# baryshnikova-lab/safepy

Measured on AMD Instinct MI355X. Metric: node-attribute enrichments/sec (nodes x attrs x perms), compute_pvalues permutation test, higher is better.
Workload: dtype u1 (bit-sliced integer counts; f64 outputs)

## Files before the change

safepy_amd/csrc/attr.hip:

```cpp
#include "common.h"

template <typename T>
__device__ __forceinline__ double load_attr(const void *raw, int64_t idx) {
    return static_cast<double>(reinterpret_cast<const T *>(raw)[idx]);
}

template <typename T, int GC>
__global__ __launch_bounds__(256) void k_attr_stats(const void *__restrict__ raw, int64_t n, int64_t m,
                                                    int64_t rs, int64_t cs, unsigned int *__restrict__ row_bits,
                                                    unsigned long long *__restrict__ acc ,
                                                    double *__restrict__ col_sum, unsigned long long *__restrict__ max_abs_bits,
                                                    unsigned int *__restrict__ col_nan, int64_t rows_per_block) {
    extern __shared__ unsigned int s_bits[];
    constexpr int RL = 256 / GC;
    const int cx = GC == 1 ? 0 : (threadIdx.x & (GC - 1));
    const int ry = GC == 1 ? threadIdx.x : (threadIdx.x / GC);
    const int lane = threadIdx.x & 63;
    const int64_t j = static_cast<int64_t>(blockIdx.x) * GC + cx;
    const int64_t n_words = (n + 31) / 32;
    __shared__ double s_sum[256];
    __shared__ double s_max[256];
    __shared__ unsigned int s_nan[256], s_other[256], s_nonint[256];
    const int64_t r_begin = static_cast<int64_t>(blockIdx.y) * rows_per_block;
    const int64_t r_end = r_begin + rows_per_block < n ? r_begin + rows_per_block : n;
// ... 134 lines not shown
        const unsigned int o = __shfl_down(mx, off);
        mx = o > mx ? o : mx;
    }
    if ((threadIdx.x & 63) == 0) s_mx[threadIdx.x >> 6] = mx;
    if (threadIdx.x < 64) {
        unsigned long long a = acc[4 + threadIdx.x], b = acc[68 + threadIdx.x];
        for (int off = 32; off; off >>= 1) {
            a += __shfl_down(a, off);
            b += __shfl_down(b, off);
        }
        if (threadIdx.x == 0) s_fold[0] = a, s_fold[1] = b;
    }
    for (int64_t i = threadIdx.x; i < n; i += 256) bytes[i] = (bits[i >> 5] >> (i & 31)) & 1u;
    __syncthreads();
    if (threadIdx.x == 0) {
        const unsigned int m01 = s_mx[0] > s_mx[1] ? s_mx[0] : s_mx[1], m23 = s_mx[2] > s_mx[3] ? s_mx[2] : s_mx[3];
        tail[0] = acc[0] = s_fold[0];
        tail[1] = acc[1] = m01 > m23 ? m01 : m23;
        tail[2] = acc[2] = s_fold[1];
        tail[3] = acc[3];
    }
}

template <typename T>
__global__ __launch_bounds__(256) void k_fill_support(const void *__restrict__ raw, int64_t n, int64_t m, int64_t rs,
                                                      int64_t cs, const int32_t *__restrict__ sup_ptr,
                                                      int32_t *__restrict__ sup_row) {
    const int64_t j = (static_cast<int64_t>(blockIdx.x) * 256 + threadIdx.x) >> 6;
    const int lane = threadIdx.x & 63;
    if (j >= m) return;
    int32_t pos = sup_ptr[j];
    for (int64_t i0 = 0; i0 < n; i0 += 64) {
        const int64_t i = i0 + lane;
        const bool one = i < n && reinterpret_cast<const T *>(raw)[i * rs + j * cs] == static_cast<T>(1);
        const unsigned long long bal = __ballot(one);
        if (one) sup_row[pos + __popcll(bal & ((1ull << lane) - 1ull))] = static_cast<int32_t>(i);
        pos += __popcll(bal);
    }
}


template <typename T>
__global__ __launch_bounds__(256) void k_reindex_rows(const T *__restrict__ table, int64_t n_labels, int64_t m,
                                                      int64_t irs, int64_t ics, const int64_t *__restrict__ row_map,
                                                      T *__restrict__ out, int64_t n, int64_t ors, int64_t ocs, T fill) {
    __shared__ T tile[64][65];
// ... 73 lines not shown
    attr->h_sup_ptr.assign(m + 1, 0);
    int64_t total = 0;
    for (int64_t j = 0; j < m; ++j) {
        total += static_cast<int64_t>(sums[j]);
        SAFE_REQUIRE(total < (1ll << 31), "attr_build_support: too many ones for int32 offsets");
        attr->h_sup_ptr[j + 1] = static_cast<int32_t>(total);
    }
    attr->n_ones = total;
    SAFE_TRY(dev_alloc(&attr->sup_ptr, m + 1));
    SAFE_TRY(dev_alloc(&attr->sup_row, total));
    SAFE_HIP_CHECK(hipMemcpyAsync(attr->sup_ptr, attr->h_sup_ptr.data(), (m + 1) * sizeof(int32_t), hipMemcpyHostToDevice,
                                  ctx->stream));
    if (attr->dtype == SAFE_DTYPE_F32)
        hipLaunchKernelGGL(k_fill_support<float>, dim3(ceil_div(m * 64, 256)), dim3(256), 0, ctx->stream, attr->raw, n, m,
                           attr->row_stride, attr->col_stride, attr->sup_ptr, attr->sup_row);
    else
        hipLaunchKernelGGL(k_fill_support<double>, dim3(ceil_div(m * 64, 256)), dim3(256), 0, ctx->stream, attr->raw, n, m,
                           attr->row_stride, attr->col_stride, attr->sup_ptr, attr->sup_row);
    SAFE_HIP_CHECK(hipGetLastError());
    return SAFE_OK;
}

static size_t flags_block_bytes(int64_t n) { return static_cast<size_t>(ceil_div(n, 8)) * 8 + 32; }

int safe_attr_prepare(safe_attr *attr) {
    if (attr->stats_ready) return SAFE_OK;
    safe_ctx *ctx = attr->ctx;
    SAFE_HIP_CHECK(hipSetDevice(ctx->device));
    const int64_t n = attr->n, m = attr->m;
    const size_t flag_bytes = flags_block_bytes(n), tail_off = flag_bytes - 32;
    const int64_t n_words = (n + 31) / 32;
    SAFE_REQUIRE(n_words * sizeof(unsigned int) <= 150 * 1024, "safe_attr_stats: too many rows for the LDS row bitmap");
    void *tmp = nullptr;
    const size_t tmp_bytes = 132 * sizeof(unsigned long long) + static_cast<size_t>(n_words + m) * sizeof(unsigned int);
    SAFE_TRY(ctx_scratch(ctx, SCRATCH_ATTR_STATS, tmp_bytes, &tmp));
    unsigned long long *d_acc = static_cast<unsigned long long *>(tmp);
    unsigned int *d_rowbits = reinterpret_cast<unsigned int *>(d_acc + 132);
    unsigned int *d_colnan = d_rowbits + n_words;
    SAFE_HIP_CHECK(hipMemsetAsync(tmp, 0, tmp_bytes, ctx->stream));
    uint8_t *flags = nullptr;
    SAFE_TRY(ctx_block_alloc(ctx, flag_bytes, reinterpret_cast<void **>(&flags)));
    if (!attr->col_sum) SAFE_TRY(ctx_block_alloc(ctx, static_cast<size_t>(m) * sizeof(double), reinterpret_cast<void **>(&attr->col_sum)));
    const bool f32 = attr->dtype == SAFE_DTYPE_F32;
    const bool c_order = attr->col_stride == 1 && m > 1;
    if (c_order) SAFE_HIP_CHECK(hipMemsetAsync(attr->col_sum, 0, m * sizeof(double), ctx->stream));
#define STATS(T, GC, RPB)                                                                                          \
    do {                                                                                                           \
        if (n_words * sizeof(unsigned int) > 32 * 1024)                                                            \
            SAFE_HIP_CHECK(hipFuncSetAttribute(reinterpret_cast<const void *>(k_attr_stats<T, GC>),                \
                                               hipFuncAttributeMaxDynamicSharedMemorySize,                         \
                                               static_cast<int>(n_words * sizeof(unsigned int))));                 \
        hipLaunchKernelGGL((k_attr_stats<T, GC>), dim3(ceil_div(m, GC), ceil_div(n, RPB)), dim3(256),              \
                           n_words * sizeof(unsigned int), ctx->stream, attr->raw, n, m, attr->row_stride,         \
                           attr->col_stride, d_rowbits, d_acc, attr->col_sum, d_acc + 3, d_colnan,                 \
                           static_cast<int64_t>(RPB));                                                             \
    } while (0)
    if (c_order) {
        const int64_t groups = ceil_div(m, 64);
        const int64_t want_chunks = std::max<int64_t>(1, 2048 / groups);
        const int64_t rpb = std::max<int64_t>(256, ceil_div(ceil_div(n, want_chunks), 64) * 64);
        if (f32) STATS(float, 64, rpb);
        else STATS(double, 64, rpb);
    } else {
        if (f32) STATS(float, 1, n);
        else STATS(double, 1, n);
    }
#undef STATS
    hipLaunchKernelGGL(k_stats_finish, dim3(1), dim3(256), 0, ctx->stream, d_acc, d_colnan, m, d_rowbits, n, flags,
                       reinterpret_cast<unsigned long long *>(flags + tail_off));
    SAFE_HIP_CHECK(hipGetLastError());
    void *pinned = nullptr;
    SAFE_TRY(ctx_pinned(ctx, flag_bytes, &pinned));
    SAFE_HIP_CHECK(hipMemcpyAsync(pinned, flags, flag_bytes, hipMemcpyDeviceToHost, ctx->stream));
    SAFE_HIP_CHECK(safe_stream_sync(ctx->stream));
    const uint8_t *h_flags = static_cast<const uint8_t *>(pinned);
    unsigned long long h_acc[4];
    memcpy(h_acc, h_flags + tail_off, sizeof(h_acc));
    attr->n_other = static_cast<int64_t>(h_acc[0]);
    attr->max_nan_col = static_cast<int64_t>(h_acc[1]);
    attr->n_non_integer = static_cast<int64_t>(h_acc[2]);
    double mx;
    memcpy(&mx, &h_acc[3], sizeof(double));
    attr->max_abs = mx;
    if (!attr->flags_ready) {
        if (attr->row_flags) ctx_block_free(ctx, attr->row_flags, flag_bytes);
        attr->row_flags = flags;
        attr->flags_ready = true;
        int64_t cnt = 0;
        for (int64_t i = 0; i < n; ++i) cnt += h_flags[i] != 0;
        attr->n_rows_with_value = cnt;
        attr->h_row_flags.assign(h_flags, h_flags + n);
    } else {
        ctx_block_free(ctx, flags, flag_bytes);
    }
    attr->stats_ready = true;
    return SAFE_OK;
}

enum : unsigned int {
    CSC_PTR_FIRST = 1u,
// ... 369 lines not shown
    SAFE_HIP_CHECK(hipMemcpyAsync(h_acc, d_acc, sizeof(h_acc), hipMemcpyDeviceToHost, ctx->stream));
    SAFE_HIP_CHECK(safe_stream_sync(ctx->stream));
    if (n_nan) *n_nan = static_cast<int64_t>(h_acc[0]);
    if (n_zero) *n_zero = static_cast<int64_t>(h_acc[1]);
    if (n_positive) *n_positive = static_cast<int64_t>(h_acc[2]);
    if (n_negative) *n_negative = static_cast<int64_t>(h_acc[3]);
    return SAFE_OK;
}

int safe_attr_nan_to_zero(safe_attr *attr) {
    SAFE_REQUIRE(attr != nullptr, "safe_attr_nan_to_zero: attr is NULL");
    safe_ctx *ctx = attr->ctx;
    SAFE_HIP_CHECK(hipSetDevice(ctx->device));
    const int64_t count = attr->n * attr->m;
    const unsigned blocks = static_cast<unsigned>(std::min<int64_t>(ceil_div(count, 256), 8192));
    void *raw = const_cast<void *>(attr->raw);
    if (attr->dtype == SAFE_DTYPE_F32)
        hipLaunchKernelGGL(k_nan_to_zero<float>, dim3(blocks), dim3(256), 0, ctx->stream, reinterpret_cast<float *>(raw), count);
    else
        hipLaunchKernelGGL(k_nan_to_zero<double>, dim3(blocks), dim3(256), 0, ctx->stream, reinterpret_cast<double *>(raw), count);
    SAFE_HIP_CHECK(hipGetLastError());
    SAFE_HIP_CHECK(safe_stream_sync(ctx->stream));
    attr->stats_ready = false;
    attr->flags_ready = false;
    attr_free_support(attr);
    return SAFE_OK;
}

int safe_attr_download(safe_attr *attr, void *out_host) {
    SAFE_REQUIRE(attr && out_host, "safe_attr_download: NULL argument");
    safe_ctx *ctx = attr->ctx;
    SAFE_HIP_CHECK(hipSetDevice(ctx->device));
    const size_t bytes = static_cast<size_t>(attr->n) * attr->m * (attr->dtype == SAFE_DTYPE_F32 ? 4 : 8);
    SAFE_HIP_CHECK(hipMemcpyAsync(out_host, attr->raw, bytes, hipMemcpyDeviceToHost, ctx->stream));
    SAFE_HIP_CHECK(safe_stream_sync(ctx->stream));
    return SAFE_OK;
}

int safe_attr_destroy(safe_attr *attr) {
    if (!attr) return SAFE_OK;
    (void)hipSetDevice(attr->ctx->device);
    (void)safe_stream_sync(attr->ctx->stream);
    if (attr->owns_raw && attr->raw_pool_bytes) ctx_block_free(attr->ctx, const_cast<void *>(attr->raw), attr->raw_pool_bytes);
    else if (attr->owns_raw) (void)dev_free(attr->raw);
    ctx_block_free(attr->ctx, attr->row_flags, flags_block_bytes(attr->n));
    ctx_block_free(attr->ctx, attr->col_sum, static_cast<size_t>(attr->m) * sizeof(double));
    attr_free_support(attr);
    delete attr;
    return SAFE_OK;
}

int safe_attr_stats(safe_attr *attr, int64_t *n_other, int64_t *max_nan_col, int64_t *n_rows_with_value,
                    int64_t *n_non_integer) {
    SAFE_REQUIRE(attr != nullptr, "safe_attr_stats: attr is NULL");
    SAFE_TRY(safe_attr_prepare(attr));
    if (n_other) *n_other = attr->n_other;
    if (max_nan_col) *max_nan_col = attr->max_nan_col;
    if (n_rows_with_value) *n_rows_with_value = attr->n_rows_with_value;
    if (n_non_integer) *n_non_integer = attr->n_non_integer;
    return SAFE_OK;
}

int safe_attr_row_flags(safe_attr *attr, uint8_t *out_host) {
    SAFE_REQUIRE(attr && out_host, "safe_attr_row_flags: NULL argument");
    SAFE_TRY(safe_attr_prepare(attr));
    if (static_cast<int64_t>(attr->h_row_flags.size()) == attr->n) {
        memcpy(out_host, attr->h_row_flags.data(), attr->n);
        return SAFE_OK;
    }
// ... 39 lines not shown
```

safepy_amd/csrc/common.h:

```cpp
#pragma once
#include <hip/hip_runtime.h>

#include <algorithm>
#include <cstdarg>
#include <cmath>
#include <cstdint>
#include <cstdio>
#include <cstdlib>
#include <cstring>
#include <condition_variable>
#include <memory>
#include <mutex>
#include <atomic>
#include <string>
#include <thread>
#include <vector>

#include "safe_hip.h"
#include "bits_plan.h"

#define SAFE_WAVE 64
#define SAFE_PAD_U16 0xFFFFu

void safe_set_error(const char *fmt, ...);
// ... 362 lines not shown
    unsigned int *enriched;
    const double *nes_table;
    double nes_threshold;
    int sign_mode;
    int mode;
    int64_t ld;
};

struct safe_attr {
    safe_ctx *ctx = nullptr;
    int64_t n = 0, m = 0;
    int dtype = SAFE_DTYPE_F64;
    int64_t row_stride = 0, col_stride = 0;
    const void *raw = nullptr;
    bool owns_raw = false;
    size_t raw_pool_bytes = 0;
    uint8_t *row_flags = nullptr;
    std::vector<uint8_t> h_row_flags;
    bool flags_ready = false;
    bool stats_ready = false;
    int64_t n_other = 0, max_nan_col = 0, n_rows_with_value = 0, n_non_integer = 0;
    double *col_sum = nullptr;
    double max_abs = 0.0;
    int32_t *sup_ptr = nullptr;
    int32_t *sup_row = nullptr;
    int64_t n_ones = 0;
    std::vector<int32_t> h_sup_ptr;
    size_t sup_ptr_pool_bytes = 0, sup_row_pool_bytes = 0;
};

struct DrawStream;

struct safe_perms {
    safe_ctx *ctx = nullptr;
    int64_t n = 0;
    int64_t count = 0;
    int64_t k = 0;
    std::vector<int32_t> h_movable;
    DrawStream *stream = nullptr;
    int64_t generated = 0, enqueued = 0;
    std::vector<int64_t> stages;
    std::vector<hipEvent_t> chunk_done;
    std::vector<uint32_t> h_local;
    std::thread drawer;
    bool on_worker = false;
    bool worker_done = false;
    bool twin = false;
    bool on_worker2 = false, worker_done2 = false;
    DrawStream *stream2 = nullptr;
    void *h_stage2[3] = {nullptr, nullptr, nullptr};
    hipEvent_t staged2[3] = {nullptr, nullptr, nullptr};
    std::vector<uint32_t> h_local2;
// ... 104 lines not shown
```

safepy_amd/csrc/enrich.hip:

```cpp
#include <algorithm>
#include <cmath>
#include <numeric>

#include "common.h"
#include "hyp_math.h"

template <typename T, int BN, int PLANES>
__global__ __launch_bounds__(256) void k_tile_prep(const void *__restrict__ raw, int64_t n, int64_t rs, int64_t cs,
                                                   int64_t col0, int64_t mloc, int64_t n_tiles,
                                                   double *__restrict__ bt) {
    const int64_t idx = static_cast<int64_t>(blockIdx.x) * 256 + threadIdx.x;
    const int64_t total = n_tiles * (n + 1) * BN;
    if (idx >= total) return;
    const int c = static_cast<int>(idx % BN);
    const int64_t row = (idx / BN) % (n + 1);
    const int64_t tile = idx / (static_cast<int64_t>(BN) * (n + 1));
    const int64_t j = tile * BN + c;
    double v = 0.0, v2 = 0.0, nn = 0.0;
    if (row < n && j < mloc) {
        const T x = reinterpret_cast<const T *>(raw)[row * rs + (col0 + j) * cs];
        if (x == x) {
            v = static_cast<double>(x);
            v2 = static_cast<double>(static_cast<T>(x * x));
            nn = 1.0;
// ... 1151 lines not shown
                                         uint32_t (&l1)[CL]) {
    blk_task_core<LV, CL, DBG>(obs, perm_ids, perm_stride, lane, nblk, np, g0, g1, l0, l1);
}

template <int LV>
__device__ __forceinline__ void observed_wave(const u32x4 *__restrict__ ids, int lane, int nblk, uint32_t *__restrict__ obs,
                                              uint32_t (&oo0)[BT_LV], uint32_t (&oo1)[BT_LV]) {
    uint32_t o0[LV], o1[LV];
    blk_sum<LV, 2, 1>(ids, lane, nblk, o0, o1);
#pragma unroll
    for (int l = 0; l < BT_LV; ++l) {
        oo0[l] = l < LV ? o0[l < LV ? l : 0] : 0u;
        oo1[l] = l < LV ? o1[l < LV ? l : 0] : 0u;
        obs[l * 64 + lane] = oo0[l];
        obs[(BT_LV + l) * 64 + lane] = oo1[l];
    }
}

__global__ __launch_bounds__(256) void k_bits_observed(int64_t n, const int32_t *__restrict__ sell_row,
                                                       const int64_t *__restrict__ slice_off,
                                                       const int32_t *__restrict__ slice_width,
                                                       const uint16_t *__restrict__ sell_col2b, int64_t n_slices,
                                                       const uint2 *__restrict__ bbits, int64_t mloc,
                                                       uint32_t *__restrict__ obs, double *__restrict__ ns_out) {
    extern __shared__ unsigned int lds[];
    uint2 *T = reinterpret_cast<uint2 *>(lds);
    if ((uint32_t)(uintptr_t)((__attribute__((address_space(3))) unsigned int *)lds) != 0u) __builtin_trap();
    const int wave = __builtin_amdgcn_readfirstlane(threadIdx.x >> 6), lane = threadIdx.x & 63;
    const int64_t wg = blockIdx.x, s = static_cast<int64_t>(blockIdx.y) * 4 + wave;
    load_word_column(T, bbits + wg * (n + 1), n);
    __syncthreads();
    if (s >= n_slices) return;
    const int wdt = __builtin_amdgcn_readfirstlane(slice_width[s]);
    const u32x4 *ids = reinterpret_cast<const u32x4 *>(sell_col2b) + slice_off[s] / 8;
    uint32_t *my_obs = obs + (wg * n_slices + s) * (2 * BT_LV * 64);
    uint32_t oo0[BT_LV], oo1[BT_LV];
    if (wdt <= 8) observed_wave<4>(ids, lane, wdt >> 3, my_obs, oo0, oo1);
    else if (wdt <= 56) observed_wave<6>(ids, lane, wdt >> 3, my_obs, oo0, oo1);
    else if (wdt <= 248) observed_wave<8>(ids, lane, wdt >> 3, my_obs, oo0, oo1);
    else if (wdt <= 504) observed_wave<9>(ids, lane, wdt >> 3, my_obs, oo0, oo1);
    else observed_wave<BT_LV>(ids, lane, wdt >> 3, my_obs, oo0, oo1);
    if (ns_out) {
        const int32_t row = sell_row[s * 64 + lane];
        uint16_t *tile = reinterpret_cast<uint16_t *>(lds + 2 * ((n + 2) & ~int64_t(1)) + 4) + wave * (64 * 66);
#pragma unroll
        for (int half = 0; half < 2; ++half)
#pragma unroll
            for (int bit = 0; bit < 32; ++bit)
                tile[lane * 66 + half * 32 + bit] = static_cast<uint16_t>(half ? vextract<BT_LV>(oo1, bit) : vextract<BT_LV>(oo0, bit));
        const int64_t jc = wg * 64 + lane;
#pragma unroll 8
        for (int r = 0; r < 64; ++r) {
// ... 327 lines not shown
    const int64_t j = wg * 64 + lane;
    bool one = false;
    if (r < n && j < mloc) one = reinterpret_cast<const T *>(raw)[r * rs + (col0 + j) * cs] == static_cast<T>(1);
    const unsigned long long w = __builtin_amdgcn_ballot_w64(one);
    if (lane == 0) bbits[wg * (n + 1) + r] = make_uint2(static_cast<uint32_t>(w), static_cast<uint32_t>(w >> 32));
}

static void launch_bits_prep(safe_ctx *ctx, const safe_attr *attr, int64_t col0, int64_t mloc, int64_t n_wg, uint2 *d_bits) {
    const int64_t n = attr->n;
    const bool f32 = attr->dtype == SAFE_DTYPE_F32;
    if (attr->col_stride == 1 && attr->row_stride != 1) {
        const dim3 grid(n_wg, ceil_div(n + 1, 4)), block(256);
        if (f32) hipLaunchKernelGGL(k_bits_prep_rowmajor<float>, grid, block, 0, ctx->stream, attr->raw, n, attr->row_stride,
                                    attr->col_stride, col0, mloc, n_wg, d_bits);
        else hipLaunchKernelGGL(k_bits_prep_rowmajor<double>, grid, block, 0, ctx->stream, attr->raw, n, attr->row_stride,
                                attr->col_stride, col0, mloc, n_wg, d_bits);
    } else {
        const dim3 grid(ceil_div(n_wg * (n + 1), 256)), block(256);
        if (f32) hipLaunchKernelGGL(k_bits_prep<float>, grid, block, 0, ctx->stream, attr->raw, n, attr->row_stride,
                                    attr->col_stride, col0, mloc, n_wg, d_bits);
        else hipLaunchKernelGGL(k_bits_prep<double>, grid, block, 0, ctx->stream, attr->raw, n, attr->row_stride,
                                attr->col_stride, col0, mloc, n_wg, d_bits);
    }
}


template <bool TABLE>
__global__ __launch_bounds__(64) void k_counts_bits(const int32_t *__restrict__ sell_row,
                                                    const int64_t *__restrict__ slice_off,
                                                    const int32_t *__restrict__ slice_width,
                                                    const int32_t *__restrict__ sell_col, int64_t n,
                                                    const uint2 *__restrict__ bbits, int64_t mloc,
                                                    double *__restrict__ out, HypLookup hl) {
    const int64_t s = blockIdx.x, wg = blockIdx.y;
    const int lane = threadIdx.x;
    const int32_t row = sell_row[s * 64 + lane];
    const int32_t *cols = sell_col + slice_off[s] + lane;
    const int wdt = slice_width[s];
    const uint2 *T = bbits + wg * (n + 1);
    uint32_t s0[BT_LV], s1[BT_LV];
#pragma unroll
    for (int l = 0; l < BT_LV; ++l) s0[l] = s1[l] = 0;
    for (int t0 = 0; t0 < wdt; t0 += 8) {
        uint32_t x0[8], x1[8];
#pragma unroll
        for (int u = 0; u < 8; ++u) {
// ... 593 lines not shown
constexpr int BITS_NS = 2;

struct BitsBuffers {
    uint2 *d_bits = nullptr;
    int4 *d_tasks = nullptr;
    unsigned int *d_queue = nullptr, *d_gl = nullptr;
    int64_t n_pad = 0, entries_pad = 0;
    uint16_t *d_ids[BITS_NS] = {nullptr, nullptr};
    uint16_t *d_ids_tail = nullptr;
    uint32_t *d_obs = nullptr;
};
static int bits_call_buffers(safe_ctx *ctx, const safe_nbr *nbr, const BitsForm &form, const BitsTail &tail, int64_t mloc, int64_t span,
                             int64_t tail_span, BitsBuffers *b) {
    const size_t n_task = bits_plan_records(nbr->bits_plan, form).size();
    const int64_t n_launch = tail.n_major + tail.n_chunks;
    void *ws = nullptr;
    SAFE_TRY(ctx_scratch(ctx, SCRATCH_TASKS, n_task * sizeof(int4) + (8 * n_launch + 4) * sizeof(unsigned int), &ws));
    b->d_tasks = static_cast<int4 *>(ws);
    b->d_queue = reinterpret_cast<unsigned int *>(b->d_tasks + n_task);
    b->n_pad = nbr->n_slices * 64;
    SAFE_TRY(ctx_scratch(ctx, SCRATCH_COUNTERS, static_cast<size_t>(b->n_pad) * mloc * sizeof(unsigned int), reinterpret_cast<void **>(&b->d_gl)));
    SAFE_HIP_CHECK(hipMemcpyAsync(b->d_tasks, nbr->bits_plan_pinned, n_task * sizeof(int4), hipMemcpyHostToDevice, ctx->stream));
    SAFE_HIP_CHECK(hipMemsetAsync(b->d_queue, 0, 8 * n_launch * sizeof(unsigned int), ctx->stream));
    SAFE_HIP_CHECK(hipMemsetAsync(b->d_gl, 0, static_cast<size_t>(b->n_pad) * mloc * sizeof(unsigned int), ctx->stream));
    safe_trace("launch_bits: buffers ready");
    b->entries_pad = (nbr->sell_entries + 1024 + 255) / 256 * 256;
    for (int s = 0; s < BITS_NS; ++s)
        SAFE_TRY(ctx_scratch(ctx, scratch_pair(SCRATCH_STREAM_A, s), static_cast<size_t>(span) * b->entries_pad * sizeof(uint16_t), reinterpret_cast<void **>(&b->d_ids[s])));
    if (tail.n_chunks)
        SAFE_TRY(ctx_scratch(ctx, SCRATCH_BITS_TAIL_IDS, static_cast<size_t>(tail_span) * b->entries_pad * sizeof(uint16_t), reinterpret_cast<void **>(&b->d_ids_tail)));
    return SAFE_OK;
}

static int bits_observe(safe_ctx *ctx, const safe_nbr *nbr, const BitsForm &form, int64_t mloc, double *ns_out, BitsBuffers *b) {
    const int64_t n_wg = ceil_div(mloc, 64);
    SAFE_TRY(ctx_scratch(ctx, SCRATCH_BITS_OBSERVED, static_cast<size_t>(n_wg) * nbr->n_slices * 2 * BT_LV * 64 * sizeof(uint32_t),
                         reinterpret_cast<void **>(&b->d_obs)));
    const size_t lds_obs = form.lds_bytes + (ns_out ? 4 * 64 * 66 * sizeof(uint16_t) : 0);
    SAFE_HIP_CHECK(hipFuncSetAttribute(reinterpret_cast<const void *>(k_bits_observed), hipFuncAttributeMaxDynamicSharedMemorySize,
                                       static_cast<int>(lds_obs)));
    hipLaunchKernelGGL(k_bits_observed, dim3(n_wg, ceil_div(nbr->n_slices, 4)), dim3(256), lds_obs, ctx->stream, nbr->n, nbr->sell_row,
                       nbr->slice_off, nbr->slice_width, nbr->sell_col2b, nbr->n_slices, b->d_bits, mloc, b->d_obs, ns_out);
    SAFE_HIP_CHECK(hipGetLastError());
    return SAFE_OK;
}

static int bits_tail_lists(safe_ctx *ctx, const safe_nbr *nbr, safe_perms *perms, const std::vector<int64_t> &starts, const BitsTail &tail,
                           const BitsBuffers &b, hipEvent_t *plain) {
    hipStream_t tail_ps = ctx->more_streams[1], kstreams[BITS_NS] = {ctx->stream, ctx->side_stream};
    const int64_t n_stage = static_cast<int64_t>(starts.size()) - 1, entries_pad = b.entries_pad;
    SAFE_HIP_CHECK(hipStreamWaitEvent(tail_ps, plain[0], 0));
    for (int64_t t = tail.n_major; t < n_stage; ++t) {
        SAFE_TRY(perms_wait(perms, starts[t + 1], tail_ps));
        hipLaunchKernelGGL(k_permute_cols, dim3(ceil_div(entries_pad, 4096), starts[t + 1] - starts[t]), dim3(256),
                           static_cast<size_t>(perms->stride16) * sizeof(uint16_t), tail_ps, perms->table16, perms->stride16,
                           nbr->sell_col2b, nbr->sell_entries, entries_pad, starts[t], starts[t + 1] - starts[t],
                           static_cast<uint32_t>(8 * nbr->n), b.d_ids_tail + (starts[t] - tail.p_split) * entries_pad, 3);
        SAFE_HIP_CHECK(hipGetLastError());
    }
    SAFE_HIP_CHECK(hipEventRecord(plain[8], tail_ps));
    for (int s = 0; s < BITS_NS; ++s) {
        SAFE_HIP_CHECK(hipEventRecord(plain[4 + s], kstreams[s]));
        SAFE_HIP_CHECK(hipStreamWaitEvent(kstreams[s], plain[8], 0));
    }
    return SAFE_OK;
// ... 37 lines not shown
        }
        const int64_t grid = std::min<int64_t>(n_tasks, grid_max);
        unsigned int *queue_c = b.d_queue + 8 * c;
        const uint16_t *ids_c = in_tail ? b.d_ids_tail : b.d_ids[c % BITS_NS];
        BitsQueues bq = blk ? plan.wave_queues[list] : plan.list_queues[list];
        void *blk_args[] = {(void *)&n, (void *)&ids_c, (void *)&entries_pad, (void *)&nbr->sell_row, (void *)&nbr->slice_off,
                            (void *)&nbr->slice_width, (void *)&b.d_obs, (void *)&nbr->n_slices, (void *)&b.d_bits, (void *)&bq,
                            (void *)&d_tasks, (void *)&p_base, (void *)&p_limit, (void *)&queue_c, (void *)&mloc, (void *)&b.d_gl,
                            (void *)&n_pad};
        void *pre_args[] = {(void *)&n, (void *)&ids_c, (void *)&entries_pad, (void *)&nbr->sell_row, (void *)&nbr->slice_off,
                            (void *)&nbr->slice_width, (void *)&nbr->sell_col2, (void *)&nbr->n_slices, (void *)&b.d_bits, (void *)&n_tasks,
                            (void *)&d_tasks, (void *)&p_base, (void *)&p_limit, (void *)&queue_c, (void *)&mloc, (void *)&b.d_gl,
                            (void *)&n_pad, (void *)&ns_out};
        SAFE_HIP_CHECK(hipLaunchKernel(kfn, dim3(grid), dim3(form.block), blk ? blk_args : pre_args, form.lds_bytes, ks));
        if (in_tail) chunk_final(c, ks);
        SAFE_HIP_CHECK(hipGetLastError());
        SAFE_HIP_CHECK(hipEventRecord(fr.ev[2 * c + 1], ks));
    }
    return SAFE_OK;
}

static int launch_bits(safe_ctx *ctx, safe_nbr *nbr, safe_attr *attr, safe_perms *perms, int64_t col0, int64_t col1,
                       const PermOut &out) {
    const int64_t n = nbr->n, mloc = col1 - col0, n_wg = ceil_div(mloc, 64), P = perms->count;
    const BitsForm form = bits_form(n, nbr->max_count, nbr->sell_col2 != nullptr, 160 * 1024);
    SAFE_REQUIRE(form.kind != BITS_NONE, "launch_bits: no bit-sliced form for %lld nodes with neighborhoods of up to %lld members",
                 static_cast<long long>(n), static_cast<long long>(nbr->max_count));
    safe_trace("launch_bits: enter");
    BitsBuffers b;
    SAFE_TRY(ctx_scratch(ctx, SCRATCH_OPERANDS, static_cast<size_t>(n_wg) * (n + 1) * sizeof(uint2), reinterpret_cast<void **>(&b.d_bits)));
    launch_bits_prep(ctx, attr, col0, mloc, n_wg, b.d_bits);
    safe_trace("launch_bits: prep launched");
    const BitsSwitches sw = bits_switches(ctx);
    int64_t span = 1;
    const std::vector<int64_t> starts = perm_launch_starts(perms, &span, 1, sw.tail_frac > 0.0);
    ctx->xc_made = 0;
    const BitsTail tail = bits_tail_split(ctx->xc_want, ctx->xc_cols, safe_ctx::XC_MAX, form.kind == BITS_BLK, starts, P, mloc, sw.tail_frac);
    const int64_t n_tail = tail.n_chunks, tail_span = P - tail.p_split;
    const int64_t n_launch = tail.n_major + n_tail;
    const int per_cu = static_cast<int>(std::max<size_t>(1, std::min<size_t>(8, (160 * 1024) / bits_lds_bytes(n, perms->stride16))));
    SAFE_TRY(bits_task_plan(ctx, nbr, form, tail, starts, static_cast<int64_t>(ctx->num_cu) * per_cu, mloc));
    safe_trace("launch_bits: tasks built");
    SAFE_TRY(bits_call_buffers(ctx, nbr, form, tail, mloc, span, tail_span, &b));
    const void *kfn = bits_form_kernel(form, sw.dbg);
    if (!kfn) return SAFE_E_INVALID;
    SAFE_HIP_CHECK(hipFuncSetAttribute(kfn, hipFuncAttributeMaxDynamicSharedMemorySize, static_cast<int>(form.lds_bytes)));
    if (form.kind == BITS_BLK) SAFE_TRY(bits_observe(ctx, nbr, form, mloc, out.ns, &b));
    for (int64_t k = 0; k < n_tail; ++k)
        if (!ctx->xc_events[k]) SAFE_HIP_CHECK(hipEventCreateWithFlags(&ctx->xc_events[k], hipEventDisableTiming));
    SpanFrame fr;
    SAFE_TRY(span_frame_open(ctx, form.kind == BITS_BLK ? "k_permtest_bits_blk" : "k_permtest_bits_pre", n_launch, 12, &fr));
    int xc_rc = SAFE_OK;
    SAFE_TRY(bits_launch_spans(ctx, nbr, perms, form, kfn, starts, tail, b, mloc, out.ns, fr, &xc_rc));
    ctx->packed_counts = b.d_gl;
// ... 3 lines not shown
    ctx->packed_layout = 0;
    SAFE_REQUIRE(xc_rc == SAFE_OK, "launch_bits: recording a column chunk's event failed");
    if (n_tail) {
        ctx->xc_made = static_cast<int>(n_tail);
        ctx->xc_tail_perms = tail_span;
        for (int64_t k = 0; k <= n_tail; ++k) ctx->xc_bounds[k] = std::min<int64_t>(k * ctx->xc_cols, mloc);
        ctx->xc_bounds[n_tail] = mloc;
        safe_trace("launch_bits: column chunks enqueued");
        if (ctx->xc_callback) ctx->xc_callback(ctx->xc_user);
    }
    SAFE_TRY(span_frame_join(ctx, fr));
    SAFE_TRY(enrich_finalize_counts(ctx, b.d_gl, b.n_pad, nbr->sell_row, mloc, P, out, nullptr));
    SAFE_HIP_CHECK(hipGetLastError());
    safe_trace("launch_bits: all enqueued");
    SAFE_TRY(span_frame_close(ctx, fr));
    safe_trace("launch_bits: synced");
    if (sw.dbg & 128) blk_trace_dump(static_cast<int>(n_launch));
    return SAFE_OK;
}

static int launch_counts_bits(safe_ctx *ctx, safe_nbr *nbr, safe_attr *attr, int64_t col0, int64_t col1, double *out_dev) {
    const int64_t n = nbr->n, mloc = col1 - col0, n_wg = ceil_div(mloc, 64);
    uint2 *d_bits = nullptr;
    SAFE_TRY(ctx_scratch(ctx, SCRATCH_OPERANDS, static_cast<size_t>(n_wg) * (n + 1) * sizeof(uint2), reinterpret_cast<void **>(&d_bits)));
    launch_bits_prep(ctx, attr, col0, mloc, n_wg, d_bits);
    SAFE_HIP_CHECK(hipEventRecord(ctx->k0, ctx->stream));
    hipLaunchKernelGGL(k_counts_bits<false>, dim3(nbr->n_slices, n_wg), dim3(64), 0, ctx->stream, nbr->sell_row, nbr->slice_off,
                       nbr->slice_width, nbr->sell_col, n, d_bits, mloc, out_dev, HypLookup{});
    SAFE_HIP_CHECK(hipGetLastError());
    SAFE_HIP_CHECK(hipEventRecord(ctx->k1, ctx->stream));
    ctx->last_kernel.name = "k_counts_bits";
    return SAFE_OK;
}

static size_t ldsf64_bytes(int64_t n, int64_t stride16) {
    return (8 * static_cast<size_t>(n + 1) + static_cast<size_t>(stride16) + 4) * sizeof(unsigned int);
}

static int launch_lds_f64(safe_ctx *ctx, safe_nbr *nbr, safe_attr *attr, safe_perms *perms, int64_t col0, int64_t col1,
                          bool z, const PermOut &out_in) {
    const int64_t n = nbr->n, mloc = col1 - col0, P = perms->count;
    const int64_t n_tiles = z ? mloc : ceil_div(mloc, 4);
    PermOut out = out_in;
    double *d_tiles = nullptr, *d_ns = out.ns;
    SAFE_TRY(ctx_scratch(ctx, SCRATCH_OPERANDS, static_cast<size_t>(n_tiles) * (n + 1) * 4 * sizeof(double), reinterpret_cast<void **>(&d_tiles)));
    if (!d_ns) SAFE_TRY(ctx_scratch(ctx, SCRATCH_F64_MATRIX, static_cast<size_t>(n) * mloc * sizeof(double), reinterpret_cast<void **>(&d_ns)));
    {
        const dim3 grid(ceil_div(n_tiles * (n + 1), 256)), block(256);
// ... 121 lines not shown
    hl.kid = d_kid;
    hl.tab = d_tab;
    hl.n_kid = n_kid;
    hl.xs = xs;
    hl.p_cut = p_cut;
    SAFE_TRY(ctx_scratch(ctx, SCRATCH_HYP_DUMMY, 64 * sizeof(double), reinterpret_cast<void **>(&hl.dummy)));
    hl.pvalues_pos = p_dev;
    hl.nes = nes_dev;
    hl.nes_binary = nb_dev;
    hl.enriched = d_enr;
    if (split) {
        int rc = mfma_counts_split_emit(ctx, nbr, split, hl);
        if (rc == SAFE_OK && enriched_f64) {
            hipLaunchKernelGGL(k_u32_to_f64, dim3(ceil_div(mloc, 256)), dim3(256), 0, ctx->stream, d_enr, enriched_f64, mloc);
            if (hipGetLastError() != hipSuccess) rc = SAFE_E_HIP;
        }
        (void)safe_stream_sync(hs);
        (void)hipEventDestroy(ids_done);
        SAFE_TRY(rc);
    } else if (use_mfma) {
        SAFE_TRY(launch_mfma_counts(ctx, nbr, attr, col0, col1, hl));
    } else {
        uint2 *d_bits = nullptr;
        SAFE_TRY(ctx_scratch(ctx, SCRATCH_OPERANDS, static_cast<size_t>(n_wg) * (n + 1) * sizeof(uint2), reinterpret_cast<void **>(&d_bits)));
        launch_bits_prep(ctx, attr, col0, mloc, n_wg, d_bits);
        SAFE_HIP_CHECK(hipEventRecord(ctx->k0, ctx->stream));
        hipLaunchKernelGGL(k_counts_bits<true>, dim3(nbr->n_slices, n_wg), dim3(64), 0, ctx->stream, nbr->sell_row, nbr->slice_off,
                           nbr->slice_width, nbr->sell_col, n, d_bits, mloc, static_cast<double *>(nullptr), hl);
        SAFE_HIP_CHECK(hipGetLastError());
        SAFE_HIP_CHECK(hipEventRecord(ctx->k1, ctx->stream));
        ctx->last_kernel.name = "k_counts_bits<hypergeom>";
    }
    if (split && enriched_f64 && enriched_done) *enriched_done = true;
    SAFE_HIP_CHECK(safe_stream_sync(ctx->stream));
    *fused = true;
    return SAFE_OK;
}

__global__ __launch_bounds__(256) void k_counts_to_outputs(const double *__restrict__ counts_neg, const double *__restrict__ counts_pos,
                                                           const double *__restrict__ ns, int64_t total, int64_t m, int64_t n_perm,
                                                           PermOut out) {
    const int64_t idx = static_cast<int64_t>(blockIdx.x) * 256 + threadIdx.x;
    if (idx >= total) return;
    const double qnan = __longlong_as_double(0x7FF8000000000000ll);
    bool obs_nan = ns && ns[idx] != ns[idx];
    const double cn = counts_neg[idx], cp = counts_pos[idx], Pd = static_cast<double>(n_perm);
    if (!obs_nan && !(cn >= 0.0 && cn <= Pd && cp >= 0.0 && cp <= Pd)) {
        atomicOr(&out.enriched[m], 1u);
// ... 545 lines not shown
```

Measured before the change: 6851 billion.

## Build attribute bit planes during stats pass and reuse them in counting kernels

Adds a kernel that, in one sweep over the raw attribute matrix, computes the column/row stats and also writes the packed 64-column bit planes used by the bit-sliced counting kernels. Those planes are cached on the attribute and reused by the counting paths, which skip their own prep pass over the raw data when the planes are valid and aligned. It also drops a separate memset of the global counter buffer by having the observed-count kernel zero it. The cost is extra device memory for the cached planes (capped at 8 MB). When non-binary values are found, the old stats kernel runs as a fallback, so the raw matrix is read twice in that case.

Measured after the change: 6900 billion, median of 6. Within noise of the previous version (+0.7%).

```diff
diff --git a/safepy_amd/csrc/attr.hip b/safepy_amd/csrc/attr.hip
--- a/safepy_amd/csrc/attr.hip
+++ b/safepy_amd/csrc/attr.hip
@@ -180,6 +180,125 @@
     }
 }
 
+template <typename T, bool ROWMAJOR>
+__global__ __launch_bounds__(256) void k_attr_planes(const T *__restrict__ raw, int64_t n, int64_t m, int64_t rs, int64_t cs,
+                                                     uint2 *__restrict__ bits, unsigned int *__restrict__ row_bits,
+                                                     unsigned long long *__restrict__ acc ,
+                                                     unsigned int *__restrict__ col_nan, unsigned int *__restrict__ col_ones) {
+    __shared__ unsigned int s_ones[64], s_nan[64];
+    const int lane = threadIdx.x & 63, wave = threadIdx.x >> 6;
+    const int64_t wg = blockIdx.x, j0 = wg * 64;
+    const int64_t r0 = static_cast<int64_t>(blockIdx.y) * 256 + wave * 64;
+    const int n_col = static_cast<int>(m - j0 < 64 ? m - j0 : 64);
+    if (threadIdx.x < 64) s_ones[threadIdx.x] = s_nan[threadIdx.x] = 0;
+    __syncthreads();
+    unsigned int my_ones = 0, my_nan = 0;
+    unsigned int n_other = 0;
+    unsigned long long has = 0;
+    uint32_t w[2] = {0, 0};
+    if (!ROWMAJOR) {
+        const int64_t r = r0 + lane;
+        const bool live = r < n;
+        bool any = false;
+        const T *src = raw + (live ? r : 0) * rs + j0 * cs;
+        auto tally = [&](int a, T x) {
+            const bool one = x == static_cast<T>(1), nan = x != x;
+            const unsigned int c1 = __popcll(__ballot(one)), cn = __popcll(__ballot(nan));
+            n_other += __popcll(__ballot(!(one || nan || x == static_cast<T>(0))));
+            if (one) (a < 32 ? w[0] : w[1]) |= 1u << (a & 31);
+            any |= live && !nan;
+            if (lane == a) my_ones += c1, my_nan += cn;
+        };
+        if (r0 < n && n_col == 64) {
+#pragma unroll
+            for (int a0 = 0; a0 < 64; a0 += 16) {
+                T x[16];
+#pragma unroll
+                for (int u = 0; u < 16; ++u) x[u] = live ? src[(a0 + u) * cs] : static_cast<T>(0);
+#pragma unroll
+                for (int u = 0; u < 16; ++u) tally(a0 + u, x[u]);
+            }
+        } else if (r0 < n) {
+            for (int a = 0; a < n_col; ++a) tally(a, live ? src[a * cs] : static_cast<T>(0));
+        }
+        has = __ballot(any);
+    } else {
+        const int64_t j = j0 + lane;
+        const bool col_live = lane < n_col;
+#pragma unroll 1
+        for (int k0 = 0; k0 < 64 && r0 + k0 < n; k0 += 16) {
+            T x[16];
+#pragma unroll
+            for (int u = 0; u < 16; ++u) {
+                const int64_t r = r0 + k0 + u;
+                x[u] = col_live && r < n ? raw[r * rs + j * cs] : static_cast<T>(0);
+            }
+#pragma unroll
+            for (int u = 0; u < 16; ++u) {
+                const int k = k0 + u;
+                const bool live = col_live && r0 + k < n;
+                const bool one = x[u] == static_cast<T>(1), nan = x[u] != x[u];
+                const unsigned long long b1 = __ballot(one);
+                n_other += __popcll(__ballot(!(one || nan || x[u] == static_cast<T>(0))));
+                if (__ballot(live && !nan)) has |= 1ull << k;
+                my_ones += one;
+                my_nan += nan;
+                if (lane == k) w[0] = static_cast<uint32_t>(b1), w[1] = static_cast<uint32_t>(b1 >> 32);
+            }
+        }
+    }
+    if (r0 + lane <= n) bits[wg * (n + 1) + r0 + lane] = make_uint2(w[0], w[1]);
+    if (lane == 0) {
+        const unsigned int lo = static_cast<unsigned int>(has), hi = static_cast<unsigned int>(has >> 32);
+        if (lo && (lo & ~row_bits[r0 >> 5])) atomicOr(&row_bits[r0 >> 5], lo);
+        if (hi && (hi & ~row_bits[(r0 >> 5) + 1])) atomicOr(&row_bits[(r0 >> 5) + 1], hi);
+        if (n_other) atomicAdd(&acc[4 + (wg & 63)], static_cast<unsigned long long>(n_other));
+    }
+    if (my_ones) atomicAdd(&s_ones[lane], my_ones);
+    if (my_nan) atomicAdd(&s_nan[lane], my_nan);
+    __syncthreads();
+    if (threadIdx.x < n_col) {
+        if (s_ones[threadIdx.x]) atomicAdd(&col_ones[j0 + threadIdx.x], s_ones[threadIdx.x]);
+        if (s_nan[threadIdx.x]) atomicAdd(&col_nan[j0 + threadIdx.x], s_nan[threadIdx.x]);
+    }
+}
+
+__global__ __launch_bounds__(256) void k_planes_finish(unsigned long long *__restrict__ acc, const unsigned int *__restrict__ col_nan,
+                                                       const unsigned int *__restrict__ col_ones, int64_t m, double *__restrict__ col_sum,
+                                                       const unsigned int *__restrict__ bits, int64_t n, uint8_t *__restrict__ bytes,
+                                                       unsigned long long *__restrict__ tail) {
+    __shared__ unsigned int s_mx[4], s_any[4];
+    __shared__ unsigned long long s_fold;
+    unsigned int mx = 0, any = 0;
+    for (int64_t i = threadIdx.x; i < m; i += 256) {
+        const unsigned int ones = col_ones[i];
+        mx = col_nan[i] > mx ? col_nan[i] : mx;
+        any |= ones;
+        col_sum[i] = static_cast<double>(ones);
+    }
+    for (int off = 32; off; off >>= 1) {
+        const unsigned int o = __shfl_down(mx, off);
+        mx = o > mx ? o : mx;
+        any |= __shfl_down(any, off);
+    }
+    if ((threadIdx.x & 63) == 0) s_mx[threadIdx.x >> 6] = mx, s_any[threadIdx.x >> 6] = any;
+    if (threadIdx.x < 64) {
+        unsigned long long a = acc[4 + threadIdx.x];
+        for (int off = 32; off; off >>= 1) a += __shfl_down(a, off);
+        if (threadIdx.x == 0) s_fold = a;
+    }
+    for (int64_t i = threadIdx.x; i < n; i += 256) bytes[i] = (bits[i >> 5] >> (i & 31)) & 1u;
+    __syncthreads();
+    if (threadIdx.x == 0) {
+        const unsigned int m01 = s_mx[0] > s_mx[1] ? s_mx[0] : s_mx[1], m23 = s_mx[2] > s_mx[3] ? s_mx[2] : s_mx[3];
+        const double mxabs = (s_any[0] | s_any[1] | s_any[2] | s_any[3]) ? 1.0 : 0.0;
+        tail[0] = acc[0] = s_fold;
+        tail[1] = acc[1] = m01 > m23 ? m01 : m23;
+        tail[2] = acc[2] = 0;
+        tail[3] = acc[3] = static_cast<unsigned long long>(__double_as_longlong(mxabs));
+    }
+}
+
 template <typename T>
 __global__ __launch_bounds__(256) void k_fill_support(const void *__restrict__ raw, int64_t n, int64_t m, int64_t rs,
                                                       int64_t cs, const int32_t *__restrict__ sup_ptr,
@@ -299,6 +418,10 @@
 }
 
 static size_t flags_block_bytes(int64_t n) { return static_cast<size_t>(ceil_div(n, 8)) * 8 + 32; }
+static size_t attr_plane_bytes(const safe_attr *attr) {
+    return static_cast<size_t>(ceil_div(attr->m, 64)) * static_cast<size_t>(attr->n + 1) * sizeof(uint2);
+}
+constexpr size_t ATTR_PLANES_POOL_MAX = size_t(8) << 20;
 
 int safe_attr_prepare(safe_attr *attr) {
     if (attr->stats_ready) return SAFE_OK;
@@ -309,50 +432,80 @@
     const int64_t n_words = (n + 31) / 32;
     SAFE_REQUIRE(n_words * sizeof(unsigned int) <= 150 * 1024, "safe_attr_stats: too many rows for the LDS row bitmap");
     void *tmp = nullptr;
-    const size_t tmp_bytes = 132 * sizeof(unsigned long long) + static_cast<size_t>(n_words + m) * sizeof(unsigned int);
+    const size_t tmp_bytes = 132 * sizeof(unsigned long long) + static_cast<size_t>(n_words + 2 * m) * sizeof(unsigned int);
     SAFE_TRY(ctx_scratch(ctx, SCRATCH_ATTR_STATS, tmp_bytes, &tmp));
     unsigned long long *d_acc = static_cast<unsigned long long *>(tmp);
     unsigned int *d_rowbits = reinterpret_cast<unsigned int *>(d_acc + 132);
     unsigned int *d_colnan = d_rowbits + n_words;
-    SAFE_HIP_CHECK(hipMemsetAsync(tmp, 0, tmp_bytes, ctx->stream));
+    unsigned int *d_colones = d_colnan + m;
     uint8_t *flags = nullptr;
     SAFE_TRY(ctx_block_alloc(ctx, flag_bytes, reinterpret_cast<void **>(&flags)));
     if (!attr->col_sum) SAFE_TRY(ctx_block_alloc(ctx, static_cast<size_t>(m) * sizeof(double), reinterpret_cast<void **>(&attr->col_sum)));
     const bool f32 = attr->dtype == SAFE_DTYPE_F32;
     const bool c_order = attr->col_stride == 1 && m > 1;
-    if (c_order) SAFE_HIP_CHECK(hipMemsetAsync(attr->col_sum, 0, m * sizeof(double), ctx->stream));
-#define STATS(T, GC, RPB)                                                                                          \
-    do {                                                                                                           \
-        if (n_words * sizeof(unsigned int) > 32 * 1024)                                                            \
-            SAFE_HIP_CHECK(hipFuncSetAttribute(reinterpret_cast<const void *>(k_attr_stats<T, GC>),                \
-                                               hipFuncAttributeMaxDynamicSharedMemorySize,                         \
-                                               static_cast<int>(n_words * sizeof(unsigned int))));                 \
-        hipLaunchKernelGGL((k_attr_stats<T, GC>), dim3(ceil_div(m, GC), ceil_div(n, RPB)), dim3(256),              \
-                           n_words * sizeof(unsigned int), ctx->stream, attr->raw, n, m, attr->row_stride,         \
-                           attr->col_stride, d_rowbits, d_acc, attr->col_sum, d_acc + 3, d_colnan,                 \
-                           static_cast<int64_t>(RPB));                                                             \
-    } while (0)
-    if (c_order) {
-        const int64_t groups = ceil_div(m, 64);
-        const int64_t want_chunks = std::max<int64_t>(1, 2048 / groups);
-        const int64_t rpb = std::max<int64_t>(256, ceil_div(ceil_div(n, want_chunks), 64) * 64);
-        if (f32) STATS(float, 64, rpb);
-        else STATS(double, 64, rpb);
-    } else {
-        if (f32) STATS(float, 1, n);
-        else STATS(double, 1, n);
-    }
-#undef STATS
-    hipLaunchKernelGGL(k_stats_finish, dim3(1), dim3(256), 0, ctx->stream, d_acc, d_colnan, m, d_rowbits, n, flags,
-                       reinterpret_cast<unsigned long long *>(flags + tail_off));
-    SAFE_HIP_CHECK(hipGetLastError());
     void *pinned = nullptr;
     SAFE_TRY(ctx_pinned(ctx, flag_bytes, &pinned));
-    SAFE_HIP_CHECK(hipMemcpyAsync(pinned, flags, flag_bytes, hipMemcpyDeviceToHost, ctx->stream));
-    SAFE_HIP_CHECK(safe_stream_sync(ctx->stream));
     const uint8_t *h_flags = static_cast<const uint8_t *>(pinned);
     unsigned long long h_acc[4];
-    memcpy(h_acc, h_flags + tail_off, sizeof(h_acc));
+    attr->bits_ready = false;
+    const size_t plane_bytes = attr_plane_bytes(attr);
+    bool swept = false;
+    if (plane_bytes <= ATTR_PLANES_POOL_MAX) {
+        if (!attr->bits) SAFE_TRY(ctx_block_alloc(ctx, plane_bytes, reinterpret_cast<void **>(&attr->bits)));
+        SAFE_HIP_CHECK(hipMemsetAsync(tmp, 0, tmp_bytes, ctx->stream));
+        const dim3 grid(static_cast<unsigned int>(ceil_div(m, 64)), static_cast<unsigned int>(ceil_div(n + 1, 256)));
+#define PLANES(T, RM)                                                                                                      \
+    hipLaunchKernelGGL((k_attr_planes<T, RM>), grid, dim3(256), 0, ctx->stream, static_cast<const T *>(attr->raw), n, m,   \
+                       attr->row_stride, attr->col_stride, attr->bits, d_rowbits, d_acc, d_colnan, d_colones)
+        if (attr->col_stride == 1 && attr->row_stride != 1) {
+            if (f32) PLANES(float, true);
+            else PLANES(double, true);
+        } else {
+            if (f32) PLANES(float, false);
+            else PLANES(double, false);
+        }
+#undef PLANES
+        hipLaunchKernelGGL(k_planes_finish, dim3(1), dim3(256), 0, ctx->stream, d_acc, d_colnan, d_colones, m, attr->col_sum, d_rowbits, n,
+                           flags, reinterpret_cast<unsigned long long *>(flags + tail_off));
+        SAFE_HIP_CHECK(hipGetLastError());
+        SAFE_HIP_CHECK(hipMemcpyAsync(pinned, flags, flag_bytes, hipMemcpyDeviceToHost, ctx->stream));
+        SAFE_HIP_CHECK(safe_stream_sync(ctx->stream));
+        memcpy(h_acc, h_flags + tail_off, sizeof(h_acc));
+        swept = h_acc[0] == 0;
+    }
+    if (!swept) {
+        SAFE_HIP_CHECK(hipMemsetAsync(tmp, 0, tmp_bytes, ctx->stream));
+        if (c_order) SAFE_HIP_CHECK(hipMemsetAsync(attr->col_sum, 0, m * sizeof(double), ctx->stream));
+#define STATS(T, GC, RPB)                                                                                          \
+        do {                                                                                                       \
+            if (n_words * sizeof(unsigned int) > 32 * 1024)                                                        \
+                SAFE_HIP_CHECK(hipFuncSetAttribute(reinterpret_cast<const void *>(k_attr_stats<T, GC>),            \
+                                                   hipFuncAttributeMaxDynamicSharedMemorySize,                     \
+                                                   static_cast<int>(n_words * sizeof(unsigned int))));             \
+            hipLaunchKernelGGL((k_attr_stats<T, GC>), dim3(ceil_div(m, GC), ceil_div(n, RPB)), dim3(256),          \
+                               n_words * sizeof(unsigned int), ctx->stream, attr->raw, n, m, attr->row_stride,     \
+                               attr->col_stride, d_rowbits, d_acc, attr->col_sum, d_acc + 3, d_colnan,             \
+                               static_cast<int64_t>(RPB));                                                         \
+        } while (0)
+        if (c_order) {
+            const int64_t groups = ceil_div(m, 64);
+            const int64_t want_chunks = std::max<int64_t>(1, 2048 / groups);
+            const int64_t rpb = std::max<int64_t>(256, ceil_div(ceil_div(n, want_chunks), 64) * 64);
+            if (f32) STATS(float, 64, rpb);
+            else STATS(double, 64, rpb);
+        } else {
+            if (f32) STATS(float, 1, n);
+            else STATS(double, 1, n);
+        }
+#undef STATS
+        hipLaunchKernelGGL(k_stats_finish, dim3(1), dim3(256), 0, ctx->stream, d_acc, d_colnan, m, d_rowbits, n, flags,
+                           reinterpret_cast<unsigned long long *>(flags + tail_off));
+        SAFE_HIP_CHECK(hipGetLastError());
+        SAFE_HIP_CHECK(hipMemcpyAsync(pinned, flags, flag_bytes, hipMemcpyDeviceToHost, ctx->stream));
+        SAFE_HIP_CHECK(safe_stream_sync(ctx->stream));
+        memcpy(h_acc, h_flags + tail_off, sizeof(h_acc));
+    }
+    attr->bits_ready = swept;
     attr->n_other = static_cast<int64_t>(h_acc[0]);
     attr->max_nan_col = static_cast<int64_t>(h_acc[1]);
     attr->n_non_integer = static_cast<int64_t>(h_acc[2]);
@@ -768,6 +921,7 @@
     SAFE_HIP_CHECK(hipGetLastError());
     SAFE_HIP_CHECK(safe_stream_sync(ctx->stream));
     attr->stats_ready = false;
+    attr->bits_ready = false;
     attr->flags_ready = false;
     attr_free_support(attr);
     return SAFE_OK;
@@ -791,6 +945,7 @@
     else if (attr->owns_raw) (void)dev_free(attr->raw);
     ctx_block_free(attr->ctx, attr->row_flags, flags_block_bytes(attr->n));
     ctx_block_free(attr->ctx, attr->col_sum, static_cast<size_t>(attr->m) * sizeof(double));
+    ctx_block_free(attr->ctx, attr->bits, attr_plane_bytes(attr));
     attr_free_support(attr);
     delete attr;
     return SAFE_OK;
diff --git a/safepy_amd/csrc/common.h b/safepy_amd/csrc/common.h
--- a/safepy_amd/csrc/common.h
+++ b/safepy_amd/csrc/common.h
@@ -408,12 +408,18 @@
     int64_t n_other = 0, max_nan_col = 0, n_rows_with_value = 0, n_non_integer = 0;
     double *col_sum = nullptr;
     double max_abs = 0.0;
+    uint2 *bits = nullptr;
+    bool bits_ready = false;
     int32_t *sup_ptr = nullptr;
     int32_t *sup_row = nullptr;
     int64_t n_ones = 0;
     std::vector<int32_t> h_sup_ptr;
     size_t sup_ptr_pool_bytes = 0, sup_row_pool_bytes = 0;
 };
+static inline uint2 *attr_bits_planes(const safe_attr *a, int64_t col0, int64_t col1) {
+    if (!a->bits_ready || !a->bits || col0 % 64 != 0 || !(col1 == a->m || col1 % 64 == 0)) return nullptr;
+    return a->bits + (col0 / 64) * (a->n + 1);
+}
 
 struct DrawStream;
 
diff --git a/safepy_amd/csrc/enrich.hip b/safepy_amd/csrc/enrich.hip
--- a/safepy_amd/csrc/enrich.hip
+++ b/safepy_amd/csrc/enrich.hip
@@ -1197,12 +1197,19 @@
                                                        const int32_t *__restrict__ slice_width,
                                                        const uint16_t *__restrict__ sell_col2b, int64_t n_slices,
                                                        const uint2 *__restrict__ bbits, int64_t mloc,
-                                                       uint32_t *__restrict__ obs, double *__restrict__ ns_out) {
+                                                       uint32_t *__restrict__ obs, double *__restrict__ ns_out,
+                                                       unsigned int *__restrict__ gl_clear) {
     extern __shared__ unsigned int lds[];
     uint2 *T = reinterpret_cast<uint2 *>(lds);
     if ((uint32_t)(uintptr_t)((__attribute__((address_space(3))) unsigned int *)lds) != 0u) __builtin_trap();
     const int wave = __builtin_amdgcn_readfirstlane(threadIdx.x >> 6), lane = threadIdx.x & 63;
     const int64_t wg = blockIdx.x, s = static_cast<int64_t>(blockIdx.y) * 4 + wave;
+    if (gl_clear && s < n_slices) {
+        const int64_t n_pad = n_slices * 64;
+        const int n_col = static_cast<int>(mloc - wg * 64 < 64 ? mloc - wg * 64 : 64);
+        unsigned int *p = gl_clear + wg * 64 * n_pad + s * 64 + lane;
+        for (int c = 0; c < n_col; ++c) p[c * n_pad] = 0u;
+    }
     load_word_column(T, bbits + wg * (n + 1), n);
     __syncthreads();
     if (s >= n_slices) return;
@@ -1576,6 +1583,15 @@
         else hipLaunchKernelGGL(k_bits_prep<double>, grid, block, 0, ctx->stream, attr->raw, n, attr->row_stride,
                                 attr->col_stride, col0, mloc, n_wg, d_bits);
     }
+}
+
+static int bits_operand(safe_ctx *ctx, const safe_attr *attr, int64_t col0, int64_t col1, uint2 **d_bits) {
+    *d_bits = attr_bits_planes(attr, col0, col1);
+    if (*d_bits) return SAFE_OK;
+    const int64_t mloc = col1 - col0, n_wg = ceil_div(mloc, 64);
+    SAFE_TRY(ctx_scratch(ctx, SCRATCH_OPERANDS, static_cast<size_t>(n_wg) * (attr->n + 1) * sizeof(uint2), reinterpret_cast<void **>(d_bits)));
+    launch_bits_prep(ctx, attr, col0, mloc, n_wg, *d_bits);
+    return SAFE_OK;
 }
 
 
@@ -2215,7 +2231,8 @@
     SAFE_TRY(ctx_scratch(ctx, SCRATCH_COUNTERS, static_cast<size_t>(b->n_pad) * mloc * sizeof(unsigned int), reinterpret_cast<void **>(&b->d_gl)));
     SAFE_HIP_CHECK(hipMemcpyAsync(b->d_tasks, nbr->bits_plan_pinned, n_task * sizeof(int4), hipMemcpyHostToDevice, ctx->stream));
     SAFE_HIP_CHECK(hipMemsetAsync(b->d_queue, 0, 8 * n_launch * sizeof(unsigned int), ctx->stream));
-    SAFE_HIP_CHECK(hipMemsetAsync(b->d_gl, 0, static_cast<size_t>(b->n_pad) * mloc * sizeof(unsigned int), ctx->stream));
+    if (form.kind != BITS_BLK)
+        SAFE_HIP_CHECK(hipMemsetAsync(b->d_gl, 0, static_cast<size_t>(b->n_pad) * mloc * sizeof(unsigned int), ctx->stream));
     safe_trace("launch_bits: buffers ready");
     b->entries_pad = (nbr->sell_entries + 1024 + 255) / 256 * 256;
     for (int s = 0; s < BITS_NS; ++s)
@@ -2233,7 +2250,7 @@
     SAFE_HIP_CHECK(hipFuncSetAttribute(reinterpret_cast<const void *>(k_bits_observed), hipFuncAttributeMaxDynamicSharedMemorySize,
                                        static_cast<int>(lds_obs)));
     hipLaunchKernelGGL(k_bits_observed, dim3(n_wg, ceil_div(nbr->n_slices, 4)), dim3(256), lds_obs, ctx->stream, nbr->n, nbr->sell_row,
-                       nbr->slice_off, nbr->slice_width, nbr->sell_col2b, nbr->n_slices, b->d_bits, mloc, b->d_obs, ns_out);
+                       nbr->slice_off, nbr->slice_width, nbr->sell_col2b, nbr->n_slices, b->d_bits, mloc, b->d_obs, ns_out, b->d_gl);
     SAFE_HIP_CHECK(hipGetLastError());
     return SAFE_OK;
 }
@@ -2317,14 +2334,13 @@
 
 static int launch_bits(safe_ctx *ctx, safe_nbr *nbr, safe_attr *attr, safe_perms *perms, int64_t col0, int64_t col1,
                        const PermOut &out) {
-    const int64_t n = nbr->n, mloc = col1 - col0, n_wg = ceil_div(mloc, 64), P = perms->count;
+    const int64_t n = nbr->n, mloc = col1 - col0, P = perms->count;
     const BitsForm form = bits_form(n, nbr->max_count, nbr->sell_col2 != nullptr, 160 * 1024);
     SAFE_REQUIRE(form.kind != BITS_NONE, "launch_bits: no bit-sliced form for %lld nodes with neighborhoods of up to %lld members",
                  static_cast<long long>(n), static_cast<long long>(nbr->max_count));
     safe_trace("launch_bits: enter");
     BitsBuffers b;
-    SAFE_TRY(ctx_scratch(ctx, SCRATCH_OPERANDS, static_cast<size_t>(n_wg) * (n + 1) * sizeof(uint2), reinterpret_cast<void **>(&b.d_bits)));
-    launch_bits_prep(ctx, attr, col0, mloc, n_wg, b.d_bits);
+    SAFE_TRY(bits_operand(ctx, attr, col0, col1, &b.d_bits));
     safe_trace("launch_bits: prep launched");
     const BitsSwitches sw = bits_switches(ctx);
     int64_t span = 1;
@@ -2374,8 +2390,7 @@
 static int launch_counts_bits(safe_ctx *ctx, safe_nbr *nbr, safe_attr *attr, int64_t col0, int64_t col1, double *out_dev) {
     const int64_t n = nbr->n, mloc = col1 - col0, n_wg = ceil_div(mloc, 64);
     uint2 *d_bits = nullptr;
-    SAFE_TRY(ctx_scratch(ctx, SCRATCH_OPERANDS, static_cast<size_t>(n_wg) * (n + 1) * sizeof(uint2), reinterpret_cast<void **>(&d_bits)));
-    launch_bits_prep(ctx, attr, col0, mloc, n_wg, d_bits);
+    SAFE_TRY(bits_operand(ctx, attr, col0, col1, &d_bits));
     SAFE_HIP_CHECK(hipEventRecord(ctx->k0, ctx->stream));
     hipLaunchKernelGGL(k_counts_bits<false>, dim3(nbr->n_slices, n_wg), dim3(64), 0, ctx->stream, nbr->sell_row, nbr->slice_off,
                        nbr->slice_width, nbr->sell_col, n, d_bits, mloc, out_dev, HypLookup{});
@@ -2543,8 +2558,7 @@
         SAFE_TRY(launch_mfma_counts(ctx, nbr, attr, col0, col1, hl));
     } else {
         uint2 *d_bits = nullptr;
-        SAFE_TRY(ctx_scratch(ctx, SCRATCH_OPERANDS, static_cast<size_t>(n_wg) * (n + 1) * sizeof(uint2), reinterpret_cast<void **>(&d_bits)));
-        launch_bits_prep(ctx, attr, col0, mloc, n_wg, d_bits);
+        SAFE_TRY(bits_operand(ctx, attr, col0, col1, &d_bits));
         SAFE_HIP_CHECK(hipEventRecord(ctx->k0, ctx->stream));
         hipLaunchKernelGGL(k_counts_bits<true>, dim3(nbr->n_slices, n_wg), dim3(64), 0, ctx->stream, nbr->sell_row, nbr->slice_off,
                            nbr->slice_width, nbr->sell_col, n, d_bits, mloc, static_cast<double *>(nullptr), hl);
```
